# nyasyamorina/font-renderer

Measured on AMD Instinct MI355X. Metric: Mpixel/s AA glyph coverage, higher is better.
Workload: dtype f32

## Files before the change

font-renderer_amd/csrc/fr_cov4.hip:

```cpp
#include "fr_c4.hpp"
#include <cstdio>
#include <type_traits>

namespace fr {

#ifdef FR_C4_STATS
__device__ unsigned long long g_c4_stats[16];
#endif
#ifdef FR_C4_ABLATE
#include "fr_cov4_ablate.inc"
#else
#define C4_ABL_LAUNCH_ONLY()
#define C4_ABL_JOB_ONLY()
#define C4_ABL_SEGLOAD_ONLY()
#define C4_ABL_SETUP_ONLY()
#define C4_ABL_EVAL_ONLY()
#define C4_ABL_SORT_ONLY()
#define C4_ABL_KEEP(k) true
#define C4_ABL_NODECODE 0
#endif
template <int WLOG, int RPL, int NS, int CAP>
struct C4Lds {
    static constexpr uint32_t LSTRIDE = c4_lstride(CAP);
    static constexpr uint32_t NCOL = (16u << WLOG) * (uint32_t)NS;
    static constexpr uint32_t PRB = 64u / (uint32_t)NS;
    static constexpr uint32_t CX = ((NCOL + 2u) * 4u + 15u) & ~15u;
    static constexpr uint32_t RCAP = 64u * RPL;
    static constexpr uint32_t REC = RCAP * (uint32_t)sizeof(Rec40);
    static constexpr uint32_t EROW = (16u << WLOG) + 16u;
    static constexpr uint32_t E = PRB * EROW;
    static constexpr uint32_t LISTS = 64u * LSTRIDE * 2u;
    static constexpr uint32_t OFF_PAIRS = LISTS;
    static constexpr uint32_t OFF_CY = OFF_PAIRS + C4_PCAP * 2u;
    static constexpr uint32_t OFF_CNT = OFF_CY + 256u;
    static constexpr uint32_t OFF_ROFF = OFF_CNT + 256u;
    static constexpr uint32_t WALK = OFF_ROFF + RCAP * 2u;
    static constexpr uint32_t WD = (CAP <= 16) ? 0u : NCOL * 2u;
    static constexpr uint32_t WAVE = (WALK > E + WD ? WALK : E + WD);
    static constexpr uint32_t OFF_WAVES = CX + REC;
    static constexpr uint32_t OFF_WCNT = OFF_WAVES + C4_WAVES * WAVE;
    static constexpr uint32_t TOTAL = OFF_WCNT + 64u;
};

__device__ __forceinline__ void c4_store_clip(unsigned char *dst, uint4 v, int m)
{
    if (m >= 16) { c4_store16(dst, v); return; }
    const uint32_t w[4] = {v.x, v.y, v.z, v.w};
#pragma unroll
    for (int i = 0; i < 16; ++i)
        if (i < m) dst[i] = (unsigned char)(w[i >> 2] >> (8 * (i & 3)));
}

template <int WLOG, int CAP, int RPL, int NS>
__global__ __launch_bounds__(64 * C4_WAVES) __attribute__((amdgpu_waves_per_eu(c4_occ(CAP, WLOG, RPL), c4_occ(CAP, WLOG, RPL))))
void cov4_kernel(const RenderArgs A)
{
    constexpr int FILL = 0;
#include "fr_cov4_kernel.inc"
}
template <int WLOG, int CAP, int RPL, int NS, int FILL>
__global__ __launch_bounds__(64 * C4_WAVES) __attribute__((amdgpu_waves_per_eu(c4_occ(CAP, WLOG, RPL), c4_occ(CAP, WLOG, RPL))))
void cov4_kernel(const RenderArgs A)
{
#include "fr_cov4_kernel.inc"
}

#ifdef FR_C4_STATS
extern "C" int fr_debug_read_c4_stats(unsigned long long *out16, int reset)
{
    hipError_t e = hipMemcpyFromSymbol(out16, HIP_SYMBOL(g_c4_stats), sizeof(g_c4_stats));
    if (e == hipSuccess && reset) {
        unsigned long long z[16] = {0};
        e = hipMemcpyToSymbol(HIP_SYMBOL(g_c4_stats), z, sizeof z);
    }
    return e == hipSuccess ? 0 : -2;
}
#endif
uint32_t cov4_wg_waves() { return C4_WAVES; }
uint32_t cov4_max_segments() { return 768u; }

template <int WLOG, int CAP, int RPL, int NS, int FILL>
static auto cov4_instance()
{
    if constexpr (FILL) return cov4_kernel<WLOG, CAP, RPL, NS, 1>;
    else return cov4_kernel<WLOG, CAP, RPL, NS>;
}

template <int WLOG, int RPL, int NS, int FILL>
static hipError_t cov4_launch_cap(const RenderArgs &a, dim3 grid, hipStream_t stream, char *name, size_t name_cap)
{
    const uint32_t kmax = (RPL == 2 && a.kmax > 16u) ? 16u : a.kmax;
    const int cap = RPL >= 16 ? 32 : (kmax <= 8 ? 8 : (kmax <= 16 ? 16 : 32));
    if (name) snprintf(name, name_cap, FILL ? "fr::cov4_kernel<%d, %d, %d, %d, 1>" : "fr::cov4_kernel<%d, %d, %d, %d>", WLOG, cap, RPL, NS);
    if (!grid.x) return hipSuccess;
    const size_t lds = (cap == 8 ? C4Lds<WLOG, RPL, NS, 8>::TOTAL : (cap == 16 ? C4Lds<WLOG, RPL, NS, 16>::TOTAL : C4Lds<WLOG, RPL, NS, 32>::TOTAL)) + a.lds_pad;
    const dim3 block(64 * C4_WAVES);
    if constexpr (RPL < 16) {
        if (cap == 8) return launch_kernel(cov4_instance<WLOG, 8, RPL, NS, FILL>(), grid, block, lds, stream, a);
        if (cap == 16) return launch_kernel(cov4_instance<WLOG, 16, RPL, NS, FILL>(), grid, block, lds, stream, a);
    }
    return launch_kernel(cov4_instance<WLOG, 32, RPL, NS, FILL>(), grid, block, lds, stream, a);
}

template <int WLOG, int NS, int FILL>
static hipError_t cov4_launch_rpl(const RenderArgs &a, uint32_t rec_cap, dim3 grid, hipStream_t stream, char *name, size_t name_cap)
{
    if (rec_cap <= 128u) return cov4_launch_cap<WLOG, 2, NS, FILL>(a, grid, stream, name, name_cap);
    if (rec_cap <= 256u) return cov4_launch_cap<WLOG, 4, NS, FILL>(a, grid, stream, name, name_cap);
    if (rec_cap > 512u) return cov4_launch_cap<WLOG, 16, NS, FILL>(a, grid, stream, name, name_cap);
    return cov4_launch_cap<WLOG, 8, NS, FILL>(a, grid, stream, name, name_cap);
}

template <int FILL>
static hipError_t cov4_launch_ns(const RenderArgs &a, uint32_t rec_cap, int ns, dim3 grid, hipStream_t stream, char *name, size_t name_cap)
{
    if (ns == 4) {
        if (a.strip_w == 256u) return cov4_launch_rpl<4, 4, FILL>(a, rec_cap, grid, stream, name, name_cap);
        if (a.strip_w == 128u) return cov4_launch_rpl<3, 4, FILL>(a, rec_cap, grid, stream, name, name_cap);
        if (a.strip_w == 64u) return cov4_launch_rpl<2, 4, FILL>(a, rec_cap, grid, stream, name, name_cap);
    } else if (ns == 2) {
        if (a.strip_w == 256u) return cov4_launch_rpl<4, 2, FILL>(a, rec_cap, grid, stream, name, name_cap);
        if (a.strip_w == 128u) return cov4_launch_rpl<3, 2, FILL>(a, rec_cap, grid, stream, name, name_cap);
        if (a.strip_w == 64u) return cov4_launch_rpl<2, 2, FILL>(a, rec_cap, grid, stream, name, name_cap);
    }
    return hipErrorInvalidValue;
}

hipError_t launch_cov4(const RenderArgs &a, uint32_t rec_cap, int ns, hipStream_t stream, bool launch, char *name, size_t name_cap, int fill)
{
    const dim3 grid(launch ? (uint32_t)((size_t)a.n_jobs * a.band_groups * a.strips) : 0u);
    if (fill) return cov4_launch_ns<1>(a, rec_cap, ns, grid, stream, name, name_cap);
    return cov4_launch_ns<0>(a, rec_cap, ns, grid, stream, name, name_cap);
}

}
```

font-renderer_amd/csrc/fr_cov4_kernel.inc:

```
    using L = C4Lds<WLOG, RPL, NS, CAP>;
    constexpr uint32_t LSTRIDE = L::LSTRIDE;
    static_assert(NS == 4 || NS == 2, "samples per axis");
    constexpr uint32_t RCAP = L::RCAP;
    constexpr uint32_t NW = C4_WAVES;
    constexpr uint32_t SW = 16u << WLOG;
    constexpr uint32_t NCOL = SW * (uint32_t)NS;
    constexpr uint32_t NWIN = 1u << WLOG;
    constexpr uint32_t PRB = L::PRB;
    constexpr int LN = (NS == 4) ? 2 : 1;
    constexpr bool SPLIT = RPL >= 8 && CAP == 32;
    extern __shared__ __align__(16) unsigned char smem[];

    const uint32_t tid = threadIdx.x, lane = tid & 63u;
    const uint32_t wave = (uint32_t)__builtin_amdgcn_readfirstlane((int)(tid >> 6));
    uint32_t bid = blockIdx.x, strip = 0, bgrp = 0;
    if (A.strips != 1u) { strip = bid % A.strips; bid /= A.strips; }
    if (A.band_groups != 1u) { bgrp = bid % A.band_groups; bid /= A.band_groups; }
    const uint32_t jidx = bid;
    C4_ABL_LAUNCH_ONLY();
    const Job job = A.jobs[jidx];
    const uint32_t x0s = strip * SW;
    const uint32_t band_first = bgrp * A.bands_per_wg;
    if (band_first * PRB >= job.h || x0s >= job.w) return;
    const uint32_t band_end = min(band_first + A.bands_per_wg, (job.h + PRB - 1u) / PRB);
    const uint32_t wlim = min(SW, job.w - x0s);
    const int phase = A.phase_center;
    const uint32_t seg0 = A.job_seg[2u * (size_t)jidx], nseg = A.job_seg[2u * (size_t)jidx + 1u];
    C4_ABL_JOB_ONLY();
    C4_ABL_SEGLOAD_ONLY();
    float *s_cxp = reinterpret_cast<float *>(smem);
    Rec40 *s_rec = reinterpret_cast<Rec40 *>(smem + L::CX);
    unsigned char *wregion = smem + L::OFF_WAVES + (size_t)wave * L::WAVE;
    uint32_t *s_wcnt = reinterpret_cast<uint32_t *>(smem + L::OFF_WCNT);

    uint32_t *const s_next_band = s_wcnt + 15;
    if (tid == 0u) *s_next_band = band_first + NW;
    const uint32_t rec_cnt = c4_setup<NW, RCAP, NS, NCOL, FILL>(A, job, seg0, nseg, x0s, phase, s_cxp, s_rec, s_wcnt, reinterpret_cast<uint32_t *>(smem + L::OFF_WAVES));
    const int32_t min_xs = job.min_x + (int32_t)x0s;
    const float jscale = job.scale * (float)NS;
    const float joff = (float)min_xs * (float)NS + (phase ? 0.5f : 0.0f) - 1.0f;
    const float ncolf = (float)NCOL;
    const bool few = RPL == 2 || rec_cnt <= 128u;
    const uint32_t per = few ? 2u : (uint32_t)RPL;
    uint32_t rra[RPL], rre[RPL];
#pragma unroll
    for (int i = 0; i < RPL; ++i) {
        const uint32_t k = per * lane + (uint32_t)i;
        const bool have = k < rec_cnt && (!few || i < 2);
        const uint32_t f = s_rec[have ? k : 0u].fr;
        rra[i] = have ? (f & 0xfffu) : 1u;
        rre[i] = have ? ((f >> 12) & 0xfffu) : 0u;
    }

    uint16_t *s_lists = reinterpret_cast<uint16_t *>(wregion);
    uint16_t *s_pairs = reinterpret_cast<uint16_t *>(wregion + L::OFF_PAIRS);
    float *s_cy = reinterpret_cast<float *>(wregion + L::OFF_CY);
    uint32_t *s_cnt = reinterpret_cast<uint32_t *>(wregion + L::OFF_CNT);
    int16_t *s_roff = reinterpret_cast<int16_t *>(wregion + L::OFF_ROFF);
    unsigned char *s_E = wregion;

    C4_ABL_SETUP_ONLY();
#if FR_DYN_BANDS
    for (uint32_t band = band_first + wave; band < band_end;
         band = (uint32_t)__builtin_amdgcn_readfirstlane((int)(lane == 0u ? atomicAdd(s_next_band, 1u) : 0u))) {
#else
    for (uint32_t band0 = band_first; band0 < band_end; band0 += NW) {
        const uint32_t band = band0 + wave;
        if (band >= band_end) break;
#endif
        const uint32_t y0 = band * PRB;
        const uint32_t row_b0 = band * 64u;
        const float cy = ((float)(job.max_y - (int32_t)(y0 + (lane >> LN))) - sub_off((int)(lane & (uint32_t)(NS - 1)), NS, phase)) / job.scale;
        uint16_t *mylist = s_lists + lane * LSTRIDE;
        auto init_lists = [&]() {
            const uint4 ones = make_uint4(0xfffdfffdu, 0xfffdfffdu, 0xfffdfffdu, 0xfffdfffdu);
#pragma unroll
            for (uint32_t q = 0; q < CAP / 8u; ++q) c4_st16<LSTRIDE>(mylist + 8u * q, ones);
            s_cnt[lane] = 0u;
        };
        init_lists();
        s_cy[lane] = cy;

        uint32_t c[RPL], off0 = 0u, tot;
        {
            uint32_t r0[RPL], csum = 0;
            {
                const uint32_t lo = row_b0, hi = row_b0 + 64u;
#pragma unroll
                for (int i = 0; i < RPL; ++i) {
                    r0[i] = max(rra[i], lo);
                    const uint32_t r1 = min(rre[i], hi);
                    c[i] = r1 > r0[i] ? r1 - r0[i] : 0u;
                    csum += c[i];
                }
            }
            const uint32_t incl = wave_incl_add(csum);
            tot = (uint32_t)__builtin_amdgcn_readlane((int)incl, 63);
            if (tot) {
                off0 = incl - csum;
                {
                    uint32_t off = off0, ro[RPL];
#pragma unroll
                    for (int i = 0; i < RPL; ++i) {
                        ro[i] = (r0[i] - row_b0 - off) & 0xffffu;
                        off += c[i];
                    }
                    if (few) *reinterpret_cast<uint32_t *>(s_roff + 2u * lane) = ro[0] | (ro[1] << 16);
                    else if constexpr (RPL == 4) *reinterpret_cast<uint2 *>(s_roff + 4u * lane) = make_uint2(ro[0] | (ro[1] << 16), ro[2] | (ro[3] << 16));
                    else if constexpr (RPL >= 8) {
#pragma unroll
                    for (int q8 = 0; q8 < RPL / 8; ++q8)
                        reinterpret_cast<uint4 *>(s_roff + (uint32_t)RPL * lane)[q8] = make_uint4(ro[8 * q8] | (ro[8 * q8 + 1] << 16), ro[8 * q8 + 2] | (ro[8 * q8 + 3] << 16),
                                                                                                  ro[8 * q8 + 4] | (ro[8 * q8 + 5] << 16), ro[8 * q8 + 6] | (ro[8 * q8 + 7] << 16));
                }
                }
            }
        }
        auto eval_pass = [&](uint32_t jlo, uint32_t jspan) {
            (void)jlo; (void)jspan;
            if (tot) {
                const uint32_t npairs = tot;
                uint32_t carry = 0u;
              for (uint32_t base = 0; base < npairs; base += (uint32_t)C4_PCAP) {
                if (C4_PCAP >= 512 || lane < C4_PCAP / 8) reinterpret_cast<uint4 *>(s_pairs)[lane] = make_uint4(0, 0, 0, 0);
                wave_lds_sync();
                {
                    uint32_t off = off0 - base;
#pragma unroll
                    for (int i = 0; i < RPL; ++i) {
                        if (c[i] && off < (uint32_t)C4_PCAP) s_pairs[off] = (uint16_t)(per * lane + (uint32_t)i + 1u);
                        off += c[i];
                    }
                }
                wave_lds_sync();
                const uint32_t nhere = min(npairs - base, (uint32_t)C4_PCAP);
                uint32_t k_cur = max(wave_incl_max((uint32_t)s_pairs[lane]), carry);
                carry = (uint32_t)__builtin_amdgcn_readlane((int)k_cur, 63);
                for (uint32_t p0 = 0; p0 < nhere && C4_ABL_KEEP(3); p0 += 64u) {
                    const uint32_t pn = min(p0 + 64u + lane, (uint32_t)C4_PCAP - 1u);
                    const uint32_t s_next = wave_incl_max((uint32_t)s_pairs[pn]);
                    {
                        const uint32_t p = base + p0 + lane, k1 = k_cur;
                        const bool livep = p < npairs;
#if C4_ABL_NODECODE
                        const uint32_t row = (p + (k1 & 1u)) & 63u;
                        const uint32_t raddr = L::CX + ((lane & 3u) + (A.n_jobs == 0xffffffffu ? k1 : 0u)) * (uint32_t)sizeof(Rec40);
#else
                        const uint32_t row = (uint32_t)((int32_t)p + (int32_t)s_roff[k1 - 1u]);
                        const uint32_t raddr = __umul24(k1, (uint32_t)sizeof(Rec40)) + (L::CX - (uint32_t)sizeof(Rec40));
#endif
                        const Rec40 r = *reinterpret_cast<const Rec40 *>(smem + raddr);
                        const float cyr = s_cy[row & 63u];
                        const unsigned long long linm = __builtin_amdgcn_sicmp((int32_t)r.fr, 0, 40 );
                        auto body = [&](auto kind) {
                            constexpr int KIND = decltype(kind)::value;
                            float num;
                            if (KIND == 2) {
                                num = cyr - r.b;
                            } else {
                                const float delta0 = cyr * r.a + r.c1 - r.c2;
                                const float delta = FILL ? __builtin_fmaxf(delta0, 0.0f) : delta0;
                                const float sq = sqrt_rn(delta);
                                const float numq = r.b + sq * r.sgn;
                                num = (KIND == 1) ? numq : c4_self(linm, cyr - r.b, numq);
                            }
                            const float t = div_by_int(num, r.a, r.rden);
                            const float xx = (r.ax * t + r.bx) * t + r.p0x;
                            uint32_t code;
                            if (KIND == 2) {
                                code = (r.fr >> 24) & 3u;
                            } else {
                                const float dy = r.a * t - r.b;
                                if (KIND == 1) code = FILL ? ((r.fr >> 24) & 3u) : ((dy > 0.0f) ? 0u : 2u);
                                else code = (dy > 0.0f) ? ((r.fr >> 26) & 3u) : ((r.fr >> 24) & 3u);
                            }
                            const float gf = __builtin_amdgcn_fmed3f(__builtin_fmaf(xx, jscale, -joff), 0.0f, ncolf);
                            int J = (int)gf;
                            {
                                const float c0 = s_cxp[J], c1 = s_cxp[J + 1];
                                const bool good = (c0 <= xx) & (xx < c1);
                                if (__builtin_expect(!good & livep, 0)) {
                                    while (s_cxp[J + 1] <= xx) ++J;
                                    while (s_cxp[J] > xx) --J;
                                }
                            }
                            bool keep = livep & (J > 0);
                            if constexpr (SPLIT) keep = livep & ((uint32_t)(J - 1) - jlo < jspan);
                            if (keep) {
                                const uint32_t pos = atomicAdd(&s_cnt[row & 63u], 1u);
                                uint16_t *rowlist = s_lists + __umul24(row & 63u, LSTRIDE);
                                rowlist[min(pos, (uint32_t)CAP)] = (uint16_t)(((uint32_t)J << 2) | code);
                            }
                        };
                        body(std::integral_constant<int, 0>{});
                    }
                    k_cur = max(s_next, carry);
                    carry = (uint32_t)__builtin_amdgcn_readlane((int)k_cur, 63);
                }
                wave_lds_sync();
              }
            }
        };
        eval_pass(0u, NCOL);
        C4_ABL_EVAL_ONLY();
        uint32_t cnt = s_cnt[lane];
        uint8_t *const out_band = reinterpret_cast<uint8_t *>(A.out) + ((size_t)job.out_y + y0) * A.out_stride + job.out_x + x0s;
        const uint32_t wx = lane & (NWIN - 1u);
        const uint32_t hlim = min(PRB, job.h - y0);
                const bool edge = __builtin_amdgcn_readfirstlane((int)((wlim < SW) | (hlim < PRB))) != 0;
        if (__ballot(cnt != 0u) == 0ull) {
            for (uint32_t yl = lane >> WLOG; yl < PRB; yl += (64u >> WLOG)) {
                const uint4 z = make_uint4(0, 0, 0, 0);
                unsigned char *dst = out_band + (size_t)yl * A.out_stride + 16u * wx;
                if (!edge) c4_store16(dst, z);
                else c4_store_clip(dst, z, yl < hlim ? (int)wlim - (int)(16u * wx) : 0);
            }
            wave_lds_sync();
            continue;
        }
        auto pull_sort = [&](uint32_t (&dd)[16], uint32_t n, bool blank, uint32_t &H, uint32_t &mx) {
#pragma unroll
            for (int q = 0; q < 4; ++q) {
                uint4 v = make_uint4(0xfffdfffdu, 0xfffdfffdu, 0xfffdfffdu, 0xfffdfffdu);
                if (q < CAP / 8 && (q == 0 || __ballot(n > (uint32_t)(8 * q)) != 0ull)) v = c4_ld16<LSTRIDE>(mylist + 8 * q);
                dd[4 * q + 0] = v.x; dd[4 * q + 1] = v.y; dd[4 * q + 2] = v.z; dd[4 * q + 3] = v.w;
            }
            if (__ballot(blank)) {
#pragma unroll
                for (int q = 0; q < 16; ++q) dd[q] = blank ? 0xfffdfffdu : dd[q];
            }
            if (CAP > 16 && __ballot(n > 16u && !blank) != 0ull) {
                packed_sort<16>(dd); H = 16u;
                mx = __ballot(n > 28u) ? 32u : (__ballot(n > 24u) ? 28u : (__ballot(n > 20u) ? 24u : 20u));
            } else if (CAP > 8 && __ballot(n > 8u && !blank) != 0ull) {
                packed_sort<8>(dd); H = 8u;
                mx = __ballot(n > 12u) ? 16u : 12u;
            } else {
                packed_sort<4>(dd); H = 4u;
                mx = __ballot(n > 4u) ? 8u : 4u;
            }
        };
        bool ovf = cnt > (uint32_t)CAP;
        uint32_t d[16];
        uint32_t Hcur, maxcnt;
        [[maybe_unused]] uint32_t dl[SPLIT ? 16 : 1];
        [[maybe_unused]] uint32_t Hl = 0u, maxl = 0u;
        [[maybe_unused]] bool split = false;
        if constexpr (SPLIT) {
#ifdef FR_C4_STATS
            const int n0 = __popcll(__ballot(ovf));
            if (lane == 0) {
                if (n0) { atomicAdd(&g_c4_stats[9], 1ull); atomicAdd(&g_c4_stats[10], (unsigned long long)n0); }
                if (n0 >= 3) { atomicAdd(&g_c4_stats[11], 1ull); atomicAdd(&g_c4_stats[12], (unsigned long long)n0); }
            }
#endif
            if (__popcll(__ballot(ovf)) >= 3) {
                split = true;
                init_lists();
                eval_pass(NCOL / 2u, NCOL / 2u);
                const uint32_t cr = s_cnt[lane];
                pull_sort(d, cr, cr > (uint32_t)CAP, Hcur, maxcnt);
                wave_lds_sync();
                init_lists();
                eval_pass(0u, NCOL / 2u);
                const uint32_t cl = s_cnt[lane];
                pull_sort(dl, cl, cl > (uint32_t)CAP, Hl, maxl);
                ovf = (cr > (uint32_t)CAP) | (cl > (uint32_t)CAP);
                if (__ballot(ovf)) {
#pragma unroll
                    for (int q = 0; q < 16; ++q) { d[q] = ovf ? 0xfffdfffdu : d[q]; dl[q] = ovf ? 0xfffdfffdu : dl[q]; }
                }
                cnt = cr + cl;
            }
        }
        if (!split) pull_sort(d, cnt, ovf, Hcur, maxcnt);
        const unsigned long long ovf_rows = __ballot(ovf);
        wave_lds_sync();
#ifdef FR_C4_STATS
        if (lane == 0) {
            atomicAdd(&g_c4_stats[0], 1ull);
            atomicAdd(&g_c4_stats[Hcur == 4u ? 1 : (Hcur == 8u ? 2 : 3)], 1ull);
            atomicAdd(&g_c4_stats[4], (unsigned long long)__popcll(ovf_rows));
        }
        {
            const uint32_t csum = wave_incl_add(cnt);
            if (lane == 63) atomicAdd(&g_c4_stats[5], (unsigned long long)csum);
            const unsigned long long g8 = __ballot(cnt > 8u), g16 = __ballot(cnt > 16u), g32 = __ballot(cnt > 32u);
            if (lane == 0) {
                atomicAdd(&g_c4_stats[6], (unsigned long long)__popcll(g8));
                atomicAdd(&g_c4_stats[7], (unsigned long long)__popcll(g16));
                atomicAdd(&g_c4_stats[8], (unsigned long long)__popcll(g32));
            }
        }
#endif

        C4_ABL_SORT_ONLY();
        {
            uint4 *z = reinterpret_cast<uint4 *>(s_E);
            const uint4 bias = make_uint4(0x10101010u, 0x10101010u, 0x10101010u, 0x10101010u);
            constexpr uint32_t NZ = L::E / 16u;
#pragma unroll
            for (uint32_t q = 0; q < (NZ + 63u) / 64u; ++q)
                if (NZ % 64u == 0u || lane + 64u * q < NZ) z[lane + 64u * q] = bias;
        }
        wave_lds_sync();
        if (C4_ABL_KEEP(2)) {
            unsigned char *erow = s_E + (lane >> LN) * L::EROW;
            int run = 0;
            bool zero = true;
            int A255 = -255, B4 = -NS, ns = -1;
            auto slot = [&](uint32_t dw, int o) {
                run += (int)((dw >> o) & 3u) - 1;
                const bool z = run == 0;
                if (z != zero) {
                    const uint32_t nib = (dw >> (o + 2)) & (uint32_t)(4 * NS - 1);
                    const int V = __mul24((int)(nib & (uint32_t)(NS - 1)), A255) + B4;
                    const uint32_t sh = (dw >> (o + LN - 1)) & 0x18u;
                    uint32_t *dwp = reinterpret_cast<uint32_t *>(erow + ((dw >> (o + LN + 2)) & 0xffcu));
                    atomicAdd(dwp, (uint32_t)V << sh);
                    const uint32_t g3 = __builtin_elementwise_sub_sat(nib, (uint32_t)(3 * NS));
                    atomicAdd(dwp + 1, (uint32_t)__mul24((int)g3, ns));
                    A255 = -A255; B4 = -B4; ns = -ns;
                }
                zero = z;
            };
            auto walk = [&](const uint32_t (&dd)[16], uint32_t H, uint32_t mx) {
#pragma unroll
                for (int gq = CAP / 8 - 1; gq >= 0; --gq) {
                    if ((uint32_t)(4 * gq) >= H || H + (uint32_t)(4 * gq) >= mx) continue;
#pragma unroll
                    for (int j = 4 * gq + 3; j >= 4 * gq; --j) slot(dd[j], 16);
                }
#pragma unroll
                for (int gq = CAP / 8 - 1; gq >= 0; --gq) {
                    if ((uint32_t)(4 * gq) >= H || (uint32_t)(4 * gq) >= mx) continue;
#pragma unroll
                    for (int j = 4 * gq + 3; j >= 4 * gq; --j) slot(dd[j], 0);
                }
            };
            walk(d, Hcur, maxcnt);
            if constexpr (SPLIT) { if (split) walk(dl, Hl, maxl); }
            if (run != 0) atomicAdd(reinterpret_cast<uint32_t *>(erow), (uint32_t)NS);
        }
        if (__builtin_expect(ovf_rows != 0ull, 0)) {
            uint32_t *s_wd = reinterpret_cast<uint32_t *>(wregion + L::E);
            static_assert(L::WD == 0u || L::WAVE >= L::E + NCOL * 2u, "no room for the winding differences of an over-full row");
            auto evaluate = [&](uint32_t k, float cy_r, int &J, uint32_t &step) {
                const Rec40 rk = s_rec[k];
                const bool lin = (int32_t)rk.fr < 0;
                const float delta0 = cy_r * rk.a + rk.c1 - rk.c2;
                const float delta = FILL ? __builtin_fmaxf(delta0, 0.0f) : delta0;
                const float num = lin ? (cy_r - rk.b) : (rk.b + sqrt_rn(delta) * rk.sgn);
                const float t = div_by_int(num, rk.a, rk.rden);
                const float xx = (rk.ax * t + rk.bx) * t + rk.p0x;
                const float dy = rk.a * t - rk.b;
                step = ((dy > 0.0f) ? ((rk.fr >> 26) & 3u) : ((rk.fr >> 24) & 3u)) - 1u;
                J = (int)__builtin_amdgcn_fmed3f(__builtin_fmaf(xx, jscale, -joff), 0.0f, ncolf);
                const float c0 = s_cxp[J], c1 = s_cxp[J + 1];
                if (__builtin_expect(!((c0 <= xx) & (xx < c1)), 0)) {
                    while (s_cxp[J + 1] <= xx) ++J;
                    while (s_cxp[J] > xx) --J;
                }
            };
            unsigned long long todo = ovf_rows;
            while (todo) {
                const uint32_t r = (uint32_t)__builtin_ctzll(todo);
                todo &= todo - 1ull;
                const float cy_r = __builtin_bit_cast(float, __builtin_amdgcn_readlane(__builtin_bit_cast(int, cy), (int)r));
                const uint32_t grow = row_b0 + r;
                unsigned long long hm[RPL];
                uint32_t total = 0u;
#pragma unroll
                for (int i = 0; i < RPL; ++i) {
                    hm[i] = __ballot(rra[i] <= grow && grow < rre[i]);
                    total += (uint32_t)__popcll(hm[i]);
                }
                int wcol[16];
                if constexpr (L::WD != 0u) {
                    for (uint32_t q = lane; q < NCOL * 2u / 16u; q += 64u)
                        reinterpret_cast<uint4 *>(s_wd)[q] = make_uint4(0x40004000u, 0x40004000u, 0x40004000u, 0x40004000u);
                    wave_lds_sync();
                    auto add = [&](uint32_t k) {
                        int J; uint32_t step;
                        evaluate(k, cy_r, J, step);
                        if (J > 0) atomicAdd(&s_wd[(uint32_t)(J - 1) >> 1], step << (16u * ((uint32_t)(J - 1) & 1u)));
                    };
                    if (__builtin_expect(total <= 128u, 1)) {
                        uint32_t fill = 0u;
                        uint32_t kd0 = 0xffffffffu, kd1 = 0xffffffffu;
#pragma unroll
                        for (int i = 0; i < RPL; ++i) {
                            if (hm[i] == 0ull) continue;
                            const bool hit = (hm[i] >> lane) & 1ull;
                            const uint32_t c = (uint32_t)__popcll(hm[i]);
                            const uint32_t below = __builtin_amdgcn_mbcnt_hi((uint32_t)(hm[i] >> 32), __builtin_amdgcn_mbcnt_lo((uint32_t)hm[i], 0u));
                            const uint32_t dst = hit ? ((fill + below) & 63u) : ((fill + c + (lane - below)) & 63u);
                            const uint32_t got = (uint32_t)__builtin_amdgcn_ds_permute((int)(dst << 2), (int)(hit ? per * lane + (uint32_t)i : 0xffffffffu));
                            const uint32_t end = fill + c;
                            kd0 = (lane >= fill && lane < end) ? got : kd0;
                            kd1 = (lane + 64u >= fill && lane + 64u < end) ? got : kd1;
                            fill = end;
                        }
                        if (kd0 != 0xffffffffu) add(kd0);
                        if (fill > 64u) { if (kd1 != 0xffffffffu) add(kd1); }
                    } else {
#pragma unroll
                        for (int i = 0; i < RPL; ++i)
                            if ((hm[i] >> lane) & 1ull) add(per * lane + (uint32_t)i);
                    }
                    wave_lds_sync();
                    int tot = 0;
                    if (16u * lane < NCOL) {
                        const uint4 lo4 = reinterpret_cast<const uint4 *>(s_wd)[2u * lane], hi4 = reinterpret_cast<const uint4 *>(s_wd)[2u * lane + 1u];
                        const uint32_t dws[8] = {lo4.x, lo4.y, lo4.z, lo4.w, hi4.x, hi4.y, hi4.z, hi4.w};
#pragma unroll
                        for (int c = 15; c >= 0; --c) {
                            tot += (int)((dws[c >> 1] >> (16 * (c & 1))) & 0xffffu) - 0x4000;
                            wcol[c] = tot;
                        }
                    } else {
#pragma unroll
                        for (int c = 0; c < 16; ++c) wcol[c] = 0;
                    }
                    const uint32_t incl = wave_incl_add((uint32_t)tot);
                    const int right = (int)((uint32_t)__builtin_amdgcn_readlane((int)incl, 63) - incl);
#pragma unroll
                    for (int c = 0; c < 16; ++c) wcol[c] += right;
                } else {
#pragma unroll
                    for (int c = 0; c < 16; ++c) wcol[c] = 0;
                    const int col0 = (int)(16u * lane);
#pragma unroll
                    for (int i = 0; i < RPL; ++i) {
                        if (hm[i] == 0ull) continue;
                        int J = 0; uint32_t step = 0u;
                        if ((hm[i] >> lane) & 1ull) evaluate(per * lane + (uint32_t)i, cy_r, J, step);
                        unsigned long long m = hm[i];
                        while (m) {
                            const int h = (int)__builtin_ctzll(m);
                            m &= m - 1ull;
                            const int n = __builtin_amdgcn_readlane(J, h) - col0;
                            const int sh = __builtin_amdgcn_readlane((int)step, h);
#pragma unroll
                            for (int c = 0; c < 16; ++c) wcol[c] += (c < n) ? sh : 0;
                        }
                    }
                }
                constexpr int PPL = 16 / NS;
                int cq[PPL];
#pragma unroll
                for (int q = 0; q < PPL; ++q) {
                    cq[q] = 0;
#pragma unroll
                    for (int c = 0; c < NS; ++c) cq[q] += (wcol[NS * q + c] != 0);
                }
                int prev = __shfl_up(cq[PPL - 1], 1);
                if (lane == 0) prev = 0;
#pragma unroll
                for (int dq = 0; dq < PPL / 4; ++dq) {
                    const int before = dq ? cq[4 * dq - 1] : prev;
                    const uint32_t val = (uint32_t)(cq[4 * dq] - before) + ((uint32_t)(cq[4 * dq + 1] - cq[4 * dq]) << 8) +
                                         ((uint32_t)(cq[4 * dq + 2] - cq[4 * dq + 1]) << 16) + ((uint32_t)(cq[4 * dq + 3] - cq[4 * dq + 2]) << 24);
                    if (16u * lane < NCOL) atomicAdd(reinterpret_cast<uint32_t *>(s_E + (r >> LN) * L::EROW) + lane * (uint32_t)(PPL / 4) + (uint32_t)dq, val);
                }
                wave_lds_sync();
            }
        }
        wave_lds_sync();

        constexpr uint32_t K1 = 0x01010101u;
        uint32_t lane_w = lane;
        asm volatile("" : "+v"(lane_w));
        const uint32_t wxw = lane_w & (NWIN - 1u);
        const unsigned char *const e_lane = s_E + (lane_w >> WLOG) * L::EROW + 16u * wxw;
        const uint32_t out_lane = (lane_w >> WLOG) * (uint32_t)A.out_stride + 16u * wxw;
        auto window_pass = [&](uint32_t it, auto clipped) {
            const uint32_t prow = (lane_w >> WLOG) + it * (64u >> WLOG);
            const uint4 e = *reinterpret_cast<const uint4 *>(e_lane + it * (64u >> WLOG) * L::EROW);
            uint32_t x0 = e.x * K1, x1 = e.y * K1, x2 = e.z * K1, x3 = e.w * K1;
            x0 -= 0x30201000u;
            x1 = x1 + __builtin_amdgcn_perm(x0, x0, 0x03030303u) - 0x40302010u;
            x2 = x2 + __builtin_amdgcn_perm(x1, x1, 0x03030303u) - 0x40302010u;
            x3 = x3 + __builtin_amdgcn_perm(x2, x2, 0x03030303u) - 0x40302010u;
            const uint32_t T = (x3 >> 24) - 16u;
            uint32_t inc = T;
            if (WLOG == 4) {
                inc += dpp<0x111>(inc);
                inc += dpp<0x112>(inc);
                inc += dpp<0x114>(inc);
                inc += dpp<0x118>(inc);
            } else {
                uint32_t s;
                s = dpp<0x111>(inc); inc += (wxw >= 1u) ? s : 0u;
                s = dpp<0x112>(inc); inc += (wxw >= 2u) ? s : 0u;
                if (WLOG == 3) { s = dpp<0x114>(inc); inc += (wxw >= 4u) ? s : 0u; }
            }
            const uint32_t cin = inc - T;
            const uint32_t cb4 = __builtin_amdgcn_perm(cin, cin, 0x00000000u);
            x0 += cb4; x1 += cb4; x2 += cb4; x3 += cb4;
            auto map4 = [](uint32_t x) -> uint32_t {
                uint32_t r;
                if (NS == 4) {
                    const uint32_t t = ((x + 0x07070707u) >> 5) & 0x01010101u;
                    const uint32_t u = 0xfefeff00u - t;
                    asm("v_lshl_add_u32 %0, %1, 4, %2" : "=v"(r) : "v"(x), "v"(u));
                } else {
                    const uint32_t t = ((x + 0x0d0d0d0du) >> 5) & 0x01010101u;
                    const uint32_t u = 0xfbfbfc00u - t;
                    asm("v_lshl_add_u32 %0, %1, 6, %2" : "=v"(r) : "v"(x), "v"(u));
                }
                return r;
            };
            const uint4 v = make_uint4(map4(x0), map4(x1), map4(x2), map4(x3));
            unsigned char *dst = (out_band + (size_t)(it * (64u >> WLOG)) * A.out_stride) + out_lane;
            if (!decltype(clipped)::value) c4_store16(dst, v);
            else c4_store_clip(dst, v, prow < hlim ? (int)wlim - (int)(16u * wxw) : 0);
        };
        if (C4_ABL_KEEP(1)) {
            if (__builtin_expect(!edge, 1)) {
#pragma unroll
                for (uint32_t it = 0; it < (PRB * NWIN) / 64u; ++it) window_pass(it, std::false_type{});
            } else {
#pragma clang loop unroll(disable)
                for (uint32_t it = 0; it < (PRB * NWIN) / 64u; ++it) window_pass(it, std::true_type{});
            }
        }
        wave_lds_sync();
    }
```

font-renderer_amd/csrc/fr_wave.hpp:

```cpp
#pragma once
#include "fr_device.hpp"

namespace fr {

template <int CTRL, int ROW_MASK = 0xf>
__device__ __forceinline__ uint32_t dpp(uint32_t x)
{
    return (uint32_t)__builtin_amdgcn_update_dpp(0, (int)x, CTRL, ROW_MASK, 0xf, false);
}
__device__ __forceinline__ uint32_t wave_incl_add(uint32_t x)
{
    x += dpp<0x111>(x);
    x += dpp<0x112>(x);
    x += dpp<0x114>(x);
    x += dpp<0x118>(x);
    x += dpp<0x142, 0xa>(x);
    x += dpp<0x143, 0xc>(x);
    return x;
}
__device__ __forceinline__ uint32_t wave_incl_max(uint32_t x)
{
    x = max(x, dpp<0x111>(x));
    x = max(x, dpp<0x112>(x));
    x = max(x, dpp<0x114>(x));
    x = max(x, dpp<0x118>(x));
    x = max(x, dpp<0x142, 0xa>(x));
    x = max(x, dpp<0x143, 0xc>(x));
    return x;
}

__device__ __forceinline__ void wave_lds_sync()
{
    __builtin_amdgcn_fence(__ATOMIC_RELEASE, "workgroup");
    __builtin_amdgcn_wave_barrier();
    __builtin_amdgcn_fence(__ATOMIC_ACQUIRE, "workgroup");
}

typedef unsigned short u16x2 __attribute__((ext_vector_type(2)));
__device__ __forceinline__ void pce(uint32_t &a, uint32_t &b)
{
    const u16x2 x = __builtin_bit_cast(u16x2, a), y = __builtin_bit_cast(u16x2, b);
    a = __builtin_bit_cast(uint32_t, __builtin_elementwise_min(x, y));
    b = __builtin_bit_cast(uint32_t, __builtin_elementwise_max(x, y));
}
template <int H>
__device__ __forceinline__ void packed_sort(uint32_t (&d)[16])
{
#pragma unroll
    for (int p = 1; p < H; p *= 2)
#pragma unroll
        for (int k = p; k >= 1; k /= 2)
#pragma unroll
            for (int j = k % p; j + k < H; j += 2 * k)
#pragma unroll
                for (int i = 0; i < k; ++i)
                    if (i + j + k < H && (i + j) / (2 * p) == (i + j + k) / (2 * p)) pce(d[i + j], d[i + j + k]);
#pragma unroll
    for (int j = 0; j < H / 2; ++j) {
        const uint32_t x = d[j], y = d[H - 1 - j];
        const uint32_t ys = __builtin_amdgcn_alignbit(y, y, 16);
        const u16x2 xv = __builtin_bit_cast(u16x2, x), yv = __builtin_bit_cast(u16x2, ys);
        const uint32_t mn = __builtin_bit_cast(uint32_t, __builtin_elementwise_min(xv, yv));
        const uint32_t mx = __builtin_bit_cast(uint32_t, __builtin_elementwise_max(xv, yv));
        d[j] = __builtin_amdgcn_perm(mx, mn, 0x05040100u);
        d[H - 1 - j] = __builtin_amdgcn_perm(mx, mn, 0x07060302u);
    }
#pragma unroll
    for (int k = H / 2; k >= 1; k /= 2)
#pragma unroll
        for (int j = 0; j < H; ++j)
            if (!(j & k)) pce(d[j], d[j + k]);
}

__device__ __forceinline__ uint32_t gray_debug(int w)
{
    const int v = w * 20 + 100;
    return (uint32_t)(v < 0 ? 0 : (v > 255 ? 255 : v));
}

}
```

Baseline: 2.493 million.

## Replace pair-index max-scan with start-bit mask and mbcnt run-list decode

Replaces the per-pair u16 owner array and the wave-wide inclusive max scan, which decoded which record each pair belongs to, with a start-of-run bitmask. Each lane now finds its run with mbcnt over two mask words, and a compact run list packs the record index with the row offset. The prefix sum also counts runs in the upper bits so the run list can be written in one pass. This removes the DPP max-scan per 64-pair step and shrinks the LDS for the pair buffer. In exchange it adds LDS atomics to set the bits, and it is limited by static asserts on the record count and the pair cap.

Result: slower. 1.958 million (-21.5%).

```diff
diff --git a/font-renderer_amd/csrc/fr_cov4.hip b/font-renderer_amd/csrc/fr_cov4.hip
--- a/font-renderer_amd/csrc/fr_cov4.hip
+++ b/font-renderer_amd/csrc/fr_cov4.hip
@@ -30,16 +30,18 @@
     static constexpr uint32_t EROW = (16u << WLOG) + 16u;
     static constexpr uint32_t E = PRB * EROW;
     static constexpr uint32_t LISTS = 64u * LSTRIDE * 2u;
-    static constexpr uint32_t OFF_PAIRS = LISTS;
-    static constexpr uint32_t OFF_CY = OFF_PAIRS + C4_PCAP * 2u;
+    static constexpr uint32_t OFF_BITS = LISTS;
+    static constexpr uint32_t OFF_CY = OFF_BITS + ((C4_PCAP / 8u + 15u) & ~15u);
     static constexpr uint32_t OFF_CNT = OFF_CY + 256u;
-    static constexpr uint32_t OFF_ROFF = OFF_CNT + 256u;
-    static constexpr uint32_t WALK = OFF_ROFF + RCAP * 2u;
+    static constexpr uint32_t OFF_RUN = OFF_CNT + 256u;
+    static_assert(RCAP <= 1024u, "a run list entry keeps the record index in 10 bits");
+    static constexpr uint32_t WALK = OFF_RUN + RCAP * 2u;
     static constexpr uint32_t WD = (CAP <= 16) ? 0u : NCOL * 2u;
     static constexpr uint32_t WAVE = (WALK > E + WD ? WALK : E + WD);
     static constexpr uint32_t OFF_WAVES = CX + REC;
     static constexpr uint32_t OFF_WCNT = OFF_WAVES + C4_WAVES * WAVE;
     static constexpr uint32_t TOTAL = OFF_WCNT + 64u;
+    static_assert(TOTAL <= 160u * 1024u / (uint32_t)c4_occ(CAP, WLOG, RPL) || WAVE == E + WD, "the walk buffers cost a workgroup per CU");
 };
 
 __device__ __forceinline__ void c4_store_clip(unsigned char *dst, uint4 v, int m)
diff --git a/font-renderer_amd/csrc/fr_cov4_kernel.inc b/font-renderer_amd/csrc/fr_cov4_kernel.inc
--- a/font-renderer_amd/csrc/fr_cov4_kernel.inc
+++ b/font-renderer_amd/csrc/fr_cov4_kernel.inc
@@ -53,10 +53,18 @@
     }
 
     uint16_t *s_lists = reinterpret_cast<uint16_t *>(wregion);
-    uint16_t *s_pairs = reinterpret_cast<uint16_t *>(wregion + L::OFF_PAIRS);
+    uint32_t *s_bits = reinterpret_cast<uint32_t *>(wregion + L::OFF_BITS);
     float *s_cy = reinterpret_cast<float *>(wregion + L::OFF_CY);
     uint32_t *s_cnt = reinterpret_cast<uint32_t *>(wregion + L::OFF_CNT);
-    int16_t *s_roff = reinterpret_cast<int16_t *>(wregion + L::OFF_ROFF);
+    uint16_t *s_run = reinterpret_cast<uint16_t *>(wregion + L::OFF_RUN);
+    const uint32_t run_off = L::OFF_WAVES + wave * L::WAVE + L::OFF_RUN;
+    uint32_t rec_off = L::CX;
+    asm volatile("" : "+s"(rec_off));
+    constexpr uint32_t CSH = 20u;
+    static_assert(64u * RCAP < (1u << CSH), "a band's pairs: 64 rows of every record");
+    static_assert(RCAP < (1u << (32u - CSH)), "a band's runs: every record");
+    static_assert(C4_PCAP % 64 == 0 && C4_PCAP / 64 <= 32, "a chunk's start bits: whole 64-bit words, one half per lane at most");
+    constexpr uint32_t NBW = (uint32_t)C4_PCAP / 64u;
     unsigned char *s_E = wregion;
 
     C4_ABL_SETUP_ONLY();
@@ -91,28 +99,20 @@
                     r0[i] = max(rra[i], lo);
                     const uint32_t r1 = min(rre[i], hi);
                     c[i] = r1 > r0[i] ? r1 - r0[i] : 0u;
-                    csum += c[i];
+                    csum += c[i] + (c[i] ? (1u << CSH) : 0u);
                 }
             }
             const uint32_t incl = wave_incl_add(csum);
-            tot = (uint32_t)__builtin_amdgcn_readlane((int)incl, 63);
+            tot = (uint32_t)__builtin_amdgcn_readlane((int)incl, 63) & ((1u << CSH) - 1u);
             if (tot) {
-                off0 = incl - csum;
-                {
-                    uint32_t off = off0, ro[RPL];
-#pragma unroll
-                    for (int i = 0; i < RPL; ++i) {
-                        ro[i] = (r0[i] - row_b0 - off) & 0xffffu;
-                        off += c[i];
-                    }
-                    if (few) *reinterpret_cast<uint32_t *>(s_roff + 2u * lane) = ro[0] | (ro[1] << 16);
-                    else if constexpr (RPL == 4) *reinterpret_cast<uint2 *>(s_roff + 4u * lane) = make_uint2(ro[0] | (ro[1] << 16), ro[2] | (ro[3] << 16));
-                    else if constexpr (RPL >= 8) {
-#pragma unroll
-                    for (int q8 = 0; q8 < RPL / 8; ++q8)
-                        reinterpret_cast<uint4 *>(s_roff + (uint32_t)RPL * lane)[q8] = make_uint4(ro[8 * q8] | (ro[8 * q8 + 1] << 16), ro[8 * q8 + 2] | (ro[8 * q8 + 3] << 16),
-                                                                                                  ro[8 * q8 + 4] | (ro[8 * q8 + 5] << 16), ro[8 * q8 + 6] | (ro[8 * q8 + 7] << 16));
-                }
+                const uint32_t excl = incl - csum;
+                off0 = excl & ((1u << CSH) - 1u);
+                uint32_t off = off0;
+                uint16_t *myrun = s_run + (excl >> CSH);
+#pragma unroll
+                for (int i = 0; i < RPL; ++i) {
+                    if (c[i]) *myrun++ = (uint16_t)(((per * lane + (uint32_t)i) << 6) | ((r0[i] - row_b0 - off) & 63u));
+                    off += c[i];
                 }
             }
         }
@@ -120,35 +120,37 @@
             (void)jlo; (void)jspan;
             if (tot) {
                 const uint32_t npairs = tot;
-                uint32_t carry = 0u;
+                uint32_t run_at = run_off;
               for (uint32_t base = 0; base < npairs; base += (uint32_t)C4_PCAP) {
-                if (C4_PCAP >= 512 || lane < C4_PCAP / 8) reinterpret_cast<uint4 *>(s_pairs)[lane] = make_uint4(0, 0, 0, 0);
+                if (lane < 2u * NBW) s_bits[lane] = 0u;
                 wave_lds_sync();
                 {
-                    uint32_t off = off0 - base;
+                    uint32_t at = off0 - 1u - base;
 #pragma unroll
                     for (int i = 0; i < RPL; ++i) {
-                        if (c[i] && off < (uint32_t)C4_PCAP) s_pairs[off] = (uint16_t)(per * lane + (uint32_t)i + 1u);
-                        off += c[i];
+                        if (c[i] && at < (uint32_t)C4_PCAP) atomicOr(s_bits + (at >> 5), 1u << (at & 31u));
+                        at += c[i];
                     }
                 }
                 wave_lds_sync();
                 const uint32_t nhere = min(npairs - base, (uint32_t)C4_PCAP);
-                uint32_t k_cur = max(wave_incl_max((uint32_t)s_pairs[lane]), carry);
-                carry = (uint32_t)__builtin_amdgcn_readlane((int)k_cur, 63);
+                static_assert(L::OFF_BITS + 256u <= L::OFF_CNT, "every lane reads a dword at the start bits");
+                const uint32_t bw = s_bits[lane];
                 for (uint32_t p0 = 0; p0 < nhere && C4_ABL_KEEP(3); p0 += 64u) {
-                    const uint32_t pn = min(p0 + 64u + lane, (uint32_t)C4_PCAP - 1u);
-                    const uint32_t s_next = wave_incl_max((uint32_t)s_pairs[pn]);
                     {
-                        const uint32_t p = base + p0 + lane, k1 = k_cur;
-                        const bool livep = p < npairs;
+                        const uint32_t wlo = (uint32_t)__builtin_amdgcn_readlane((int)bw, (int)(p0 >> 5));
+                        const uint32_t whi = (uint32_t)__builtin_amdgcn_readlane((int)bw, (int)(p0 >> 5) + 1);
+                        const uint32_t kr = wave_rank_below(wlo, whi);
+                        const bool livep = wave_lanes_below(nhere - p0);
 #if C4_ABL_NODECODE
-                        const uint32_t row = (p + (k1 & 1u)) & 63u;
-                        const uint32_t raddr = L::CX + ((lane & 3u) + (A.n_jobs == 0xffffffffu ? k1 : 0u)) * (uint32_t)sizeof(Rec40);
+                        const uint32_t row = (lane + (kr & 1u)) & 63u;
+                        const uint32_t raddr = L::CX + ((lane & 3u) + (A.n_jobs == 0xffffffffu ? kr : 0u)) * (uint32_t)sizeof(Rec40);
 #else
-                        const uint32_t row = (uint32_t)((int32_t)p + (int32_t)s_roff[k1 - 1u]);
-                        const uint32_t raddr = __umul24(k1, (uint32_t)sizeof(Rec40)) + (L::CX - (uint32_t)sizeof(Rec40));
+                        const uint32_t ent = *reinterpret_cast<const uint16_t *>(smem + (run_at + 2u * kr));
+                        const uint32_t row = lane + ent;
+                        const uint32_t raddr = __umul24(ent >> 6, (uint32_t)sizeof(Rec40)) + rec_off;
 #endif
+                        run_at += 2u * wave_word_bits(wlo, whi);
                         const Rec40 r = *reinterpret_cast<const Rec40 *>(smem + raddr);
                         const float cyr = s_cy[row & 63u];
                         const unsigned long long linm = __builtin_amdgcn_sicmp((int32_t)r.fr, 0, 40 );
@@ -194,8 +196,6 @@
                         };
                         body(std::integral_constant<int, 0>{});
                     }
-                    k_cur = max(s_next, carry);
-                    carry = (uint32_t)__builtin_amdgcn_readlane((int)k_cur, 63);
                 }
                 wave_lds_sync();
               }
diff --git a/font-renderer_amd/csrc/fr_wave.hpp b/font-renderer_amd/csrc/fr_wave.hpp
--- a/font-renderer_amd/csrc/fr_wave.hpp
+++ b/font-renderer_amd/csrc/fr_wave.hpp
@@ -27,6 +27,20 @@
     x = max(x, dpp<0x142, 0xa>(x));
     x = max(x, dpp<0x143, 0xc>(x));
     return x;
+}
+
+__device__ __forceinline__ uint32_t wave_rank_below(uint32_t lo, uint32_t hi)
+{
+    return __builtin_amdgcn_mbcnt_hi(hi, __builtin_amdgcn_mbcnt_lo(lo, 0u));
+}
+__device__ __forceinline__ uint32_t wave_word_bits(uint32_t lo, uint32_t hi)
+{
+    return (uint32_t)__builtin_popcount(lo) + (uint32_t)__builtin_popcount(hi);
+}
+__device__ __forceinline__ bool wave_lanes_below(uint32_t n)
+{
+    const unsigned long long m = n >= 64u ? ~0ull : ~(~0ull << n);
+    return __builtin_amdgcn_inverse_ballot_w64(m);
 }
 
 __device__ __forceinline__ void wave_lds_sync()
```
